# JeffWang987/MVSTER

Hardware: AMD Instinct MI355X
Metric: depth-maps/sec (DTU 512×640, 5-view, 4-stage) at 1/2/4/8 MI355X (higher is better)
Workload: dtype f32; 1 GPU; DTU mid 512x640, 5 views, 4-stage cascade 8/8/4/4 hyp, B=1 eval, 1 depth map(s) per step per GPU; launch=hipGraph replay, parallelism=replicas x1, depth_maps_in_flight_per_gpu=2

## Files before the change

include/mvster_hip.h:

```cpp
#ifndef MVSTER_HIP_H
#define MVSTER_HIP_H

#ifdef __cplusplus
extern "C" {
#endif

#define MVSTER_OK 0
#define MVSTER_ERR_NULL (-1)
#define MVSTER_ERR_SHAPE (-2)
#define MVSTER_ERR_UNSUPPORTED (-3)
#define MVSTER_ERR_LAUNCH (-4)

int mvster_relative_projection(const float* proj_matrices, float* rt, int B, int N, void* stream);

int mvster_relative_projection_multi(const float* const* proj_matrices, int nstage, float* rt, int B, int N,
                                     void* stream);

int mvster_pack_images(const float* const* imgs, int N, float* out, int B, int H, int W, void* stream);

int mvster_pack_images_u8(const unsigned char* imgs, float* out, int V, int H, int W, void* stream);

int mvster_load_pack_images_u8(const unsigned char* buf, long buf_bytes, const int* desc_host, const int* desc, const void* tables,
                               long table_words, float* out, unsigned char* out_u8, int V, int Hd, int Wd, void* stream);

// ... 59 lines not shown
                            float* partial, int B, int D, int h, int w, int CF, void* stream);

int mvster_upsample_bilinear(const float* in, float* out, int B, int hi, int wi, int ho, int wo, void* stream);

int mvster_upsample_bilinear_multi(const float* const* ins, float* const* outs, const int* his, const int* wis, int n, int B,
                                   int ho, int wo, void* stream);

int mvster_conv_mfma(const float* in, const float* wpk, const float* scale, const float* shift, const float* skip,
                     const float* zeros, const float* prob_w, const float* prob_b, float* out, const int* geom,
                     int ngeom, const long* woff, int cin, int mt, int nt, int variant, void* stream);

int mvster_conv_small(const float* in, const float* w, const float* scale, const float* shift, const float* skip,
                      float* out, int NB, int H, int W, int cin, int relu, void* stream);

int mvster_conv_narrow(const float* in, const float* w, const float* scale, const float* shift, const float* skip,
                       float* out, int NB, int H, int W, int cin, int relu, int mt, int wpc, void* stream);

int mvster_conv_narrow4(const float* in, const float* w, const float* scale, const float* shift, float* out, int NB, int H,
                        int W, int relu, int mt, int wpc, void* stream);

int mvster_conv_narrow_pair(const float* in, const float* w1, const float* scale1, const float* shift1, const float* w2,
                            const float* scale2, const float* shift2, float* out, int NB, int H, int W, int relu1, int relu2,
                            int wpc, void* stream);

int mvster_deconv_small(const float* in, const float* w, const float* scale, const float* shift, const float* skip,
                        const float* prob_w, const float* prob_b, float* out, int NB, int Hi, int Wi, int cin,
                        int cout, int relu, void* stream);

int mvster_deconv_select(const float* in, const float* w, const float* scale, const float* shift, const float* skip,
                         const float* prob_w, const float* prob_b, const float* hypo, float* attn, float* depth, float* conf,
                         float* inv_min, float* inv_max, float* logits_out, int B, int D, int Hi, int Wi, int cin, int relu,
                         float split_itv, void* stream);

int mvster_fpn_tail_gather(const float* G, const float* vb, float* P, float* workspace, int NB, int H, int W,
                           int CO, void* stream);

int mvster_fpn_tail_gather_bwd(const float* gP, float* gG, int NB, int H, int W, int CO, int pitch, void* stream);

int mvster_fpn_lateral_up(const float* x, const float* A, const float* bias, const float* q, float* out, int NB,
                          int H, int W, int CI, int CO, void* stream);

int mvster_fpn_tail_fused(const float* x, const float* A, const float* bias, const float* q, const float* vb, float* P,
                          int NB, int H, int W, int CI, void* stream);

int mvster_pack_conv_weights(const float* w, float* wpk, int cout, int cin, int cin_pad, int kd, int kh, int kw, long s_n,
                             long s_c, long s_z, long s_y, long s_x, int flip, void* stream);
// ... 128 lines not shown
```

mvster_amd/_lib.py:

```python
import ctypes
import os

_HERE = os.path.dirname(os.path.abspath(__file__))
LIB_PATH = os.environ.get("MVSTER_LIB") or os.path.join(_HERE, "csrc", "libmvster_hip.so")

ERR_NULL, ERR_SHAPE, ERR_UNSUPPORTED, ERR_LAUNCH = -1, -2, -3, -4
ERRORS = {-1: "NULL pointer", -2: "bad shape", -3: "unsupported channel/tile combination", -4: "kernel launch failed"}

_f = ctypes.c_void_p
_i = ctypes.c_int
_l = ctypes.c_long
_fl = ctypes.c_float

SIGNATURES = {
    "mvster_relative_projection": [_f, _f, _i, _i, _f],
    "mvster_relative_projection_multi": [_f, _i, _f, _i, _i, _f],
    "mvster_pack_images": [_f, _i, _f, _i, _i, _i, _f],
    "mvster_pack_images_u8": [_f, _f, _i, _i, _i, _f],
    "mvster_load_pack_images_u8": [_f, _l, _f, _f, _f, _l, _f, _f, _i, _i, _i, _f],
    "mvster_forward_prologue": [_f, _i, _f, _i, _i, _i, _f, _i, _f, _f, _i, _f, _i, _i, _i, _i, _f],
    "mvster_warp_agg_fwd": [_f, _f, _f, _f, _f, _f] + [_i] * 9 + [_l] * 3 + [_i, _i, _fl, _i, _f],
    "mvster_warp_agg_fwd_indexed": [_f, _f, _f, _f, _f, _f] + [_i] * 10 + [_fl, _i, _f],
    "mvster_warp_agg_fwd_counted": [_f, _f, _f, _f, _f, _f] + [_i] * 9 + [_l] * 3 + [_i, _i, _fl, _i, _f, _f],
    "mvster_warp_agg_fwd_indexed_counted": [_f, _f, _f, _f, _f, _f] + [_i] * 10 + [_fl, _i, _f, _f],
    "mvster_gather_views": [_f, _f, _f, _i, _i, _i, _l, _f],
    "mvster_warp_agg_fwd_sched": [_f] * 6 + [_i, _f, _f, _f] + [_i] * 9 + [_l] * 3 + [_i, _fl, _i, _f],
    "mvster_warp_agg_bwd": [_f] * 11 + [_i] * 9 + [_l] * 3 + [_i, _i, _fl, _f],
    "mvster_warp_agg_bwd_scratch": [_i] * 8 + [_f, _f],
    "mvster_warp_agg_bwd_sorted_scratch": [_i] * 8 + [_f, _f],
    "mvster_warp_agg_bwd_sorted": [_f] * 11 + [_i] * 9 + [_l] * 3 + [_i, _i, _fl, _f],
    "mvster_init_range": [_f, _i, _f, _i, _i, _i, _i, _i, _f],
    "mvster_schedule_inverse_range": [_f, _f, _f, _i, _i, _i, _i, _f],
    "mvster_schedule_range": [_f, _f, _f, _i, _i, _i, _i, _f],
    "mvster_select_depth": [_f, _f, _f, _f, _i, _f, _f, _f, _f, _f, _f, _f, _i, _i, _i, _i, _fl, _f],
    "mvster_select_depth_bwd": [_f, _f, _f, _f, _f, _f, _i, _i, _i, _i, _i, _f],
    "mvster_upsample_bilinear": [_f, _f, _i, _i, _i, _i, _i, _f],
    "mvster_upsample_bilinear_multi": [_f, _f, _f, _f, _i, _i, _i, _i, _f],
    "mvster_conv_mfma": [_f, _f, _f, _f, _f, _f, _f, _f, _f, _f, _i, _f, _i, _i, _i, _i, _f],
    "mvster_conv_small": [_f, _f, _f, _f, _f, _f, _i, _i, _i, _i, _i, _f],
    "mvster_conv_narrow": [_f, _f, _f, _f, _f, _f, _i, _i, _i, _i, _i, _i, _i, _f],
    "mvster_conv_narrow4": [_f, _f, _f, _f, _f, _i, _i, _i, _i, _i, _i, _f],
    "mvster_conv_narrow_pair": [_f, _f, _f, _f, _f, _f, _f, _f, _i, _i, _i, _i, _i, _i, _f],
    "mvster_deconv_select": [_f] * 14 + [_i] * 6 + [_fl, _f],
    "mvster_deconv_small": [_f, _f, _f, _f, _f, _f, _f, _f, _i, _i, _i, _i, _i, _i, _f],
    "mvster_fpn_tail_gather": [_f, _f, _f, _f, _i, _i, _i, _i, _f],
    "mvster_fpn_lateral_up": [_f, _f, _f, _f, _f, _i, _i, _i, _i, _i, _f],
    "mvster_fpn_tail_fused": [_f, _f, _f, _f, _f, _f, _i, _i, _i, _i, _f],
    "mvster_fpn_tail_gather_bwd": [_f, _f, _i, _i, _i, _i, _i, _f],
    "mvster_pack_conv_weights": [_f, _f] + [_i] * 6 + [_l] * 5 + [_i, _f],
    "mvster_pack_wino_weights": [_f, _f, _i, _i, _i, _i, _l, _l, _l, _l, _l, _i, _f],
    "mvster_pack_wino_batch": [_f, _i, _i, _f],
    "mvster_pack_conv_weights_classes": [_f, _f, _i, _i, _i, _i, _i, _f, _f, _f, _f],
    "mvster_conv_wgrad": [_f, _f, _f] + [_i] * 20 + [_f],
    "mvster_conv_wgrad_slots": [_i] * 12,
    "mvster_bn_relu_fwd": [_f, _f, _f, _f, _f, _l, _i, _i, _i, _f],
    "mvster_conv_wgrad_finish": [_f, _f] + [_i] * 10 + [_f],
    "mvster_bn_slots": [_l, _i, _i],
    "mvster_col_sum": [_f, _f, _f, _f, _l, _i, _f],
    "mvster_bn_train_slots": [_l, _i, _i],
    "mvster_bn_train_fwd": [_f] * 10 + [_l, _i, _i, _i, _fl, _fl, _f],
    "mvster_bn_train_bwd": [_f] * 7 + [_l, _i, _i, _i, _f],
    "mvster_conv_wgrad_finish_batch": [_f, _i, _f],
    "mvster_bn_relu_bwd_reduce": [_f] * 11 + [_l, _i, _i, _i, _f],
    "mvster_bn_relu_bwd_apply": [_f] * 8 + [_l, _i, _i, _i, _i, _f],
    "mvster_upsample2x_cl_fwd": [_f, _f, _i, _i, _i, _i, _f],
    "mvster_upsample2x_cl_bwd": [_f, _f, _i, _i, _i, _i, _f],
    "mvster_upsample2x_nearest_cl": [_f, _f, _i, _i, _i, _i, _i, _f],
    "mvster_sinkhorn": [_f, _f, _f, _f, _f, _i, _i, _l, _i, _fl, _f],
    "mvster_sinkhorn_continuous": [_f, _f, _f, _f, _f, _f, _i, _i, _l, _i, _fl, _f],
    "mvster_stage_loss_terms": [_f, _f, _f, _f, _f, _f, _i, _i, _l, _i, _f],
# ... 63 lines not shown
```

mvster_amd/conv_plan.py:

```python
import ctypes

import numpy as np
import torch

from . import _lib, ops

GEOM = ("B", "Di", "Hi", "Wi", "Do", "Ho", "Wo", "DoF", "HoF", "WoF", "sd", "sh", "sw", "cout", "ntile_total", "relu",
        "skip_mode", "osd", "osh", "osw", "nclass")
GEOM_CLASS = ("kd", "kh", "kw", "pd", "ph", "pw", "od", "oh", "ow", "nsteps")

SKIP_NONE, SKIP_ADD, SKIP_UPSAMPLE_ADD = 0, 1, 2


def _pack_gemm(wk):
    K, N = wk.shape
    Kp, Np = (K + 15) // 16 * 16, (N + 15) // 16 * 16
    full = wk.new_zeros(Kp, Np)
    full[:K, :N] = wk
    return full.view(Kp // 16, 4, 4, Np // 16, 16).permute(0, 3, 1, 4, 2).contiguous().view(-1), Kp // 16


def fold_bn(bn, cout, device):
    if bn is None:
        return torch.ones(cout, device=device), torch.zeros(cout, device=device)
# ... 48 lines not shown
    return _FAMILIES


def tuned_choice(layer, B, Di, Hi, Wi, skip_mode):
    import math
    sig = layer_signature(layer, B, Di, Hi, Wi, skip_mode)
    hit = _tuning().get(sig)
    if hit:
        return hit, "exact"
    if skip_mode == SKIP_ADD:
        hit = _tuning().get(sig[:-1] + "0")
        if hit:
            return hit, "exact (without skip)"
    lst = _families().get((sig[:sig.index("_", sig.index("_s") + 1)], skip_mode))
    if lst:
        lv, ld, lb = math.log2(max(1, B * Di * Hi * Wi)), math.log2(max(1, Di)), math.log2(max(1, B))
        d, val = min(((abs(e[0] - lv) + abs(e[1] - ld) + 0.25 * abs(e[2] - lb), e[3]) for e in lst), key=lambda t: t[0])
        if d <= FAMILY_REACH:
            return list(val), "family"
    return None, None


FUSE_TAIL = True
FUSE_SELECT = True
LDS_BUDGET = 12 * 256 * 16
FORCE_VARIANT = None
TPERS16_MIN_VOXELS = 40960
FUSE_CONV0 = True
NARROW_PAIR_WPC = 1
NARROW_PAIR_MIN_PIXELS = 512 * 14 * 64
NARROW_MIN_VOXELS = 64 * 256


def _lds_plan(B, Do, Ho, Wo, kernel, stride, ntile_total):
    kd, kh, kw = kernel
    if kw not in (3, 5) or Wo < 24:
        return None
    for mt in (4, 2):
        ty = 2 * mt
        patch = kd * ((ty - 1) * stride[1] + kh) * (31 * stride[2] + kw) * 64
        if patch > LDS_BUDGET or (mt == 4 and Ho < 6):
            continue
        blocks = -(-Wo // 32) * -(-Ho // ty) * Do * B
        nt = max(n for n in (4, 2, 1) if n <= ntile_total and ntile_total % n == 0)
        while nt > 1 and blocks * (ntile_total // nt) < 512:
            nt //= 2
# ... 578 lines not shown
        w3 = m.inner3.weight.detach().double()[:, :, 0, 0]
        b3 = m.inner3.bias.detach().double()
        self.tail_g, self.tail_c, self.tail_vb, wg4 = self._reassociate(m.out4, w3, b3)
        self.tail_a = (wg4 @ w2).float().contiguous()
        self.tail_ab = (wg4 @ b2).float().contiguous()

    @staticmethod
    def _reassociate(out, wi, bi):
        wo = out.weight.detach().double()
        co = wo.shape[0]
        wg = wo.permute(2, 3, 0, 1).reshape(9 * co, wo.shape[1])
        wc = torch.einsum("ocyx,ci->oiyx", wo, wi)
        g = ConvLayer(wg.float().reshape(9 * co, wo.shape[1], 1, 1), False, (1, 1), (0, 0))
        c = ConvLayer(wc.float(), False, (1, 1), (1, 1), bias=out.bias)
        vb = torch.einsum("ocyx,c->yxo", wo, bi).reshape(9, co).float().contiguous()
        return g, c, vb, wg

    @staticmethod
    def _seq(layers, x):
        for l in layers:
            x = l(x)
        return x

    def trunk(self, x):
        c0 = self._conv0(x)
        c1 = self._seq(self.conv1, c0)
        c2 = self._seq(self.conv2, c1)
        c3 = self._seq(self.conv3, c2)
        f1 = self.inner1(c2, skip=c3, skip_mode=SKIP_UPSAMPLE_ADD)
        return c0, c1, c3, f1

    def _conv0(self, x):
        a, b = self.conv0
        N, D, H, W, _ = x.shape
        if (FUSE_CONV0 and FORCE_VARIANT is None and a.w_small is not None and b.w_small is not None and a.cin == 4 and b.cin == 8
                and D == 1 and N * H * W >= NARROW_PAIR_MIN_PIXELS and x.is_cuda and a.w_small.device == x.device and x.is_contiguous() and x.dtype == torch.float32
                and hasattr(_lib.load(), "mvster_conv_narrow_pair")):
            out = torch.empty((N, 1, H, W, 8), device=x.device, dtype=torch.float32)
            rc = _lib.load().mvster_conv_narrow_pair(
                x.data_ptr(), a.w_small.data_ptr(), a.scale.data_ptr(), a.shift.data_ptr(), b.w_small.data_ptr(),
                b.scale.data_ptr(), b.shift.data_ptr(), out.data_ptr(), N, H, W, int(a.relu), int(b.relu), NARROW_PAIR_WPC, ops._stream())
            _lib.check(rc, "conv_narrow_pair")
            return out
        return self._seq(self.conv0, x)

    def coarse(self, c3, f1):
        return self.out1(c3), self.out2(f1)

    def head(self, x):
        c0, c1, c3, f1 = self.trunk(x)
        o1, o2 = self.coarse(c3, f1)
        return c0, c1, f1, o1, o2

    def tail(self, c0, c1, f1):
        return self.tail_mid(c0, c1, f1), self.tail_fine(c0, c1, f1)

    def tail_mid(self, c0, c1, f1):
        H, W = c0.shape[2], c0.shape[3]
        p3 = ops.fpn_tail_gather(self.mid_g(f1), self.mid_vb, H // 2, W // 2)
        return self.mid_c(c1, skip=p3, skip_mode=SKIP_ADD)

    def tail_fine(self, c0, c1, f1):
        H, W = c0.shape[2], c0.shape[3]
        q4 = self.tail_g(f1)
        p4 = ops.fpn_tail_fused(c1, self.tail_a, self.tail_ab, q4, self.tail_vb, H, W) if FUSE_TAIL else None
        if p4 is None:
            p4 = ops.fpn_tail_gather(ops.fpn_lateral_up(c1, self.tail_a, self.tail_ab, q4), self.tail_vb, H, W)
        return self.tail_c(c0, skip=p4, skip_mode=SKIP_ADD)

    def __call__(self, x):
        c0, c1, f1, o1, o2 = self.head(x)
        o3, o4 = self.tail(c0, c1, f1)
        return [o1, o2, o3, o4]
```

mvster_amd/csrc/conv_pers.hip:

```cpp
#include "conv_args.hpp"

namespace mvconv {
namespace {


#ifdef MVSTER_TIMELINE
__device__ unsigned long long* g_ptl = nullptr;
#define MV_PTL(k)                                                                                                       \
    do {                                                                                                                \
        __builtin_amdgcn_sched_barrier(0);                                                                              \
        if (g_ptl && lane == 0 && it < 16)                                                                              \
            g_ptl[(((size_t)(blockIdx.y * gridDim.x + blockIdx.x) * 4 + wave) * 16 + it) * 8 + (k)] =                    \
                (k) < 5 ? __builtin_amdgcn_s_memtime() : (k) == 5 ? __builtin_amdgcn_s_getreg(63492)                    \
                                                         : (k) == 6 ? __builtin_amdgcn_s_getreg(63508) : tile;          \
        __builtin_amdgcn_sched_barrier(0);                                                                              \
    } while (0)
#define MV_PPTL(k, v)                                                                                                   \
    do {                                                                                                                \
        __builtin_amdgcn_sched_barrier(0);                                                                              \
        if (g_ptl && lane == 0 && hp < 16)                                                                              \
            g_ptl[(((size_t)(blockIdx.y * gridDim.x + blockIdx.x) * 8 + wave8) * 16 + hp) * 4 + (k)] = (v);           \
        __builtin_amdgcn_sched_barrier(0);                                                                              \
    } while (0)
#else
// ... 977 lines not shown
                    const f32x4v k = __builtin_bit_cast(f32x4v, __builtin_amdgcn_raw_buffer_load_b128(skip_rsrc, off, 0, 0));
#pragma unroll
                    for (int j = 0; j < 4; ++j) v[j] += k[j];
                } else if (a.skip_mode == 2) {
                    const bool ok = n0 < (unsigned)a.cout && vox[mt] < mtot;
                    const unsigned c4 = n0 * 4u;
                    const f32x4v k00 = __builtin_bit_cast(f32x4v, __builtin_amdgcn_raw_buffer_load_b128(skip_rsrc, ok ? up[mt].o00 + c4 : 0x80000000u, 0, 0));
                    const f32x4v k01 = __builtin_bit_cast(f32x4v, __builtin_amdgcn_raw_buffer_load_b128(skip_rsrc, ok ? up[mt].o01 + c4 : 0x80000000u, 0, 0));
                    const f32x4v k10 = __builtin_bit_cast(f32x4v, __builtin_amdgcn_raw_buffer_load_b128(skip_rsrc, ok ? up[mt].o10 + c4 : 0x80000000u, 0, 0));
                    const f32x4v k11 = __builtin_bit_cast(f32x4v, __builtin_amdgcn_raw_buffer_load_b128(skip_rsrc, ok ? up[mt].o11 + c4 : 0x80000000u, 0, 0));
#pragma unroll
                    for (int j = 0; j < 4; ++j) v[j] = mv::bilerp(up[mt].ly, up[mt].lx, k00[j], k01[j], k10[j], k11[j]) + v[j];
                }
                __builtin_amdgcn_raw_buffer_store_b128(__builtin_bit_cast(u32x4v, v), out_rsrc, off, 0, MV_STORE_AUX);
            }
#pragma unroll
            for (int c = 0; c < NCH; ++c) Bv[c] = Bn[c];
        }
#pragma unroll
        for (int mt = 0; mt < MT; ++mt) {
            vox[mt] = voxn[mt];
#pragma unroll
            for (int c = 0; c < NCH; ++c) A[mt][c] = An[mt][c];
        }
    }
}


template <int MT, int NT, int KW, int SW, int NCH, int KD, bool WREG, int PF, bool SKIP, bool LD>
int launch_pers(const ConvArgs& a, int wpc, hipStream_t s) {
    using G = PersGeom<MT, KW, SW, KD>;
    constexpr int NTAP = KD * KW * KW;
    const size_t lds = (size_t)(2 * NCH * 2 * G::PLANE + 64 + (WREG ? 0 : NTAP * NCH * NT * 64)) * 16;
    if (lds > 160 * 1024) return MVSTER_ERR_UNSUPPORTED;
    auto kern = conv_pers_kernel<MT, NT, KW, SW, NCH, KD, WREG, PF, SKIP, LD>;
    static unsigned long attr_done = 0;
    if (lds > 64 * 1024 && !allow_big_lds(reinterpret_cast<const void*>(kern), attr_done)) return MVSTER_ERR_LAUNCH;
    const int g_num_cu = num_cus();
    if (g_num_cu <= 0) return MVSTER_ERR_LAUNCH;
    PersArgs p;
    if (!fill_pers_args(a, G::TY, p)) return MVSTER_ERR_UNSUPPORTED;
    const long ntiles = p.ntiles;
    p.prio = (wpc >> 4) & 1;
    wpc &= 15;
    int by_lds = (int)((160 * 1024) / lds);
    int per_cu = wpc > 0 ? wpc : (by_lds > 3 ? 3 : by_lds);
// ... 211 lines not shown
    if (mt == MT_ && nt == NT_ && kw == KW_ && sw == SW_ && nch == NCH_ && kd == KD_) {                            \
        if (ld) {                                                                                                  \
              \
            if constexpr (SW_ == 2)                                                                                \
                return a.skip_mode == 1 ? launch_pers<MT_, NT_, KW_, SW_, NCH_, KD_, WREG_, PF_, true, true>(a, wpc, s)   \
                                        : launch_pers<MT_, NT_, KW_, SW_, NCH_, KD_, WREG_, PF_, false, true>(a, wpc, s); \
            return MVSTER_ERR_UNSUPPORTED;                                                                         \
        }                                                                                                          \
        return a.skip_mode == 1 ? launch_pers<MT_, NT_, KW_, SW_, NCH_, KD_, WREG_, PF_, true, false>(a, wpc, s)   \
                                : launch_pers<MT_, NT_, KW_, SW_, NCH_, KD_, WREG_, PF_, false, false>(a, wpc, s);  \
    }
    MV_P(1, 3, 1, 1, 1, true, 2)
    MV_P(2, 3, 1, 2, 1, false, 1)
    MV_P(1, 3, 1, 2, 1, false, 1)
    MV_P(1, 3, 1, 4, 1, false, 1)
    MV_P(2, 5, 2, 1, 1, false, 1)
    MV_P(1, 3, 1, 1, 3, false, 2)
    MV_P(2, 3, 2, 1, 1, false, 1)
#undef MV_P
#undef MV_Q
    return MVSTER_ERR_UNSUPPORTED;
}

}
```

mvster_amd/graph.py:

```python
import collections

import torch


def _sample_layout(imgs, proj_matrices, depth_values):
    segs, off = [], 0
    for name, t in ([("img%d" % i, t) for i, t in enumerate(imgs)] + [("proj_" + k, proj_matrices[k]) for k in sorted(proj_matrices)]
                    + [("depth_values", depth_values)]):
        segs.append((name, off, tuple(t.shape)))
        off += (t.numel() + 63) // 64 * 64
    return segs, off


def pack_sample(imgs, proj_matrices, depth_values, pin=True):
    segs, total = _sample_layout(imgs, proj_matrices, depth_values)
    flat = torch.zeros(total, dtype=torch.float32)
    if pin:
        flat = flat.pin_memory()
    src = {("img%d" % i): t for i, t in enumerate(imgs)}
    src.update({"proj_" + k: v for k, v in proj_matrices.items()})
    src["depth_values"] = depth_values
    for name, off, shape in segs:
        flat[off:off + src[name].numel()].copy_(src[name].reshape(-1).float().cpu())
    return flat
# ... 116 lines not shown
        torch._foreach_copy_(new, self._src)
        out = {}
        for path, j in self._paths:
            if len(path) == 1:
                out[path[0]] = new[j]
            else:
                out.setdefault(path[0], {})[path[1]] = new[j]
        return {k: out[k] for k in self.outputs}


class ForwardCache:

    def __init__(self, capacity=4):
        self.capacity = capacity
        self.entries = collections.OrderedDict()
        self.stats = {"eager": 0, "captured": 0, "replayed": 0, "capture_failed": 0}
        self.disabled_keys = set()

    @staticmethod
    def key(model, imgs, proj_matrices, depth_values):
        im = imgs[0]
        from . import conv_plan, ops
        glob = (conv_plan.FORCE_VARIANT, conv_plan.FUSE_TAIL, conv_plan.FUSE_CONV0, conv_plan.NARROW_PAIR_WPC, conv_plan.FUSE_SELECT, conv_plan.LDS_BUDGET, conv_plan.NARROW_MIN_VOXELS,
                id(conv_plan._TUNING), ops.WGRAD_MAX_SLOTS)
        cfg = (glob, model.warp_variant, getattr(model, "fuse_hypotheses", None), getattr(model, "merge_launches", None), model.overlap_streams, float(model.attn_temp), model.attn_fuse_d, model.num_stage,
               tuple(model.stage_splits), tuple(model.depth_interals_ratio), tuple(model.group_cor_dim))
        return (im.device.index, len(imgs), tuple(im.shape), int(depth_values.shape[1]), tuple(sorted(proj_matrices.keys())), cfg)

    def clear(self):
        self.entries.clear()

    def __call__(self, model, imgs, proj_matrices, depth_values):
        key = self.key(model, imgs, proj_matrices, depth_values)
        if key in self.disabled_keys:
            self.stats["eager"] += 1
            return model._forward_eval(imgs, proj_matrices, depth_values)
        stamp = model._state_stamp()
        hit = self.entries.get(key)
        if hit is not None and hit[0] == stamp:
            self.entries.move_to_end(key)
            if hit[1] is None:
                try:
                    hit[1] = _CachedForward(model, imgs, proj_matrices, depth_values)
                    self.stats["captured"] += 1
                except RuntimeError as e:
                    import warnings
                    warnings.warn("mvster_amd: hipGraph capture of the eval forward failed for %r (%s): this shape stays on "
# ... 302 lines not shown
```

mvster_amd/net.py:

```python
import contextlib

import torch
import torch.nn as nn
import torch.nn.functional as F

from . import ops
from .conv_plan import FpnPlan, Reg2dPlan, Reg3dPlan
from .modules import FPN4, mono_depth_decoder, reg2d, reg3d


class _WarpAggPyr(torch.autograd.Function):

    @staticmethod
    def forward(ctx, pyr, B, rt, hypo, G, group_cor, attn_fuse_d, attn_temp):
        pyr = pyr.contiguous()
        ref_cl, src_cl = _WarpAggPyr._parts(pyr, B)
        out, wsum = ops.warp_agg_fwd_cl(ref_cl, src_cl, rt, hypo, G, group_cor, attn_fuse_d, attn_temp, want_wsum=True)
        ctx.save_for_backward(pyr, rt, hypo, out, wsum)
        ctx.cfg = (B, G, group_cor, attn_fuse_d, attn_temp)
        ctx.set_materialize_grads(False)
        return out, pyr[:B]

    @staticmethod
    def _parts(pyr, B):
        n, _, h, w, C = pyr.shape
        return pyr[:B].view(B, h, w, C), pyr[B:].view(n // B - 1, B, h, w, C)

    @staticmethod
    def backward(ctx, grad, grad_ref_maps):
# ... 196 lines not shown
                               "column)" % (tuple(depth_values.shape), B))
        if not imgs[0].is_cuda:
            raise RuntimeError("mvster_amd.MVS4net runs on MI355X only: move the model and inputs to the GPU "
                               "(there is no CPU fallback; the CPU oracle lives in oracle/ for tests)")

    @torch.no_grad()
    def _forward_eval(self, imgs, proj_matrices, depth_values, teacher=None, capture=None):
        N = len(imgs)
        B, _, H, W = imgs[0].shape
        dev = imgs[0].device
        fpn, regs = self._get_plans()
        depth_values = depth_values.to(dev, torch.float32)
        depth_interval = None
        if not self.inverse_depth:
            depth_interval = (depth_values[:, -1] - depth_values[:, 0]) / depth_values.size(1)
        names = ["stage%d" % (s + 1) for s in range(self.num_stage)]
        pms = [proj_matrices[n].to(dev, torch.float32) for n in names]
        hypo0 = None
        if self.merge_launches and (teacher is None or "stage1" not in teacher) and not self.fuse_hypotheses:
            packed, rts, hypo0 = ops.forward_prologue(imgs, pms, depth_values, self.stage_splits[0], H // 8, W // 8,
                                                      self.inverse_depth)
        else:
            packed, rts = ops.pack_images(imgs), ops.relative_projection_multi(pms)
        c0, c1, c3, f1 = fpn.trunk(packed)
        main = torch.cuda.current_stream()
        side = None
        if self.overlap_streams and self.num_stage > 2:
            side = self._side_streams.get(dev)
            if side is None:
                side = self._side_streams[dev] = torch.cuda.Stream(device=dev)
            side.wait_stream(main)
            with torch.cuda.stream(side):
                o3, o4 = fpn.tail(c0, c1, f1)
            o1, o2 = fpn.coarse(c3, f1)
        else:
            o1, o2 = fpn.coarse(c3, f1)
            o3, o4 = fpn.tail(c0, c1, f1) if self.num_stage > 2 else (None, None)
        join = None
        if side is not None:
            def join():
                main.wait_stream(side)
                if not torch.cuda.is_current_stream_capturing():
                    for t in (o3, o4):
                        t.record_stream(main)
        return self._cascade_eval([o1, o2, o3, o4], regs, N, B, H, W, rts, depth_values, depth_interval, hypo0=hypo0,
                                  teacher=teacher, capture=capture, join=join)

    @torch.no_grad()
    def _cascade_eval(self, pyramid, regs, N, B, H, W, rts, depth_values, depth_interval, hypo0=None, teacher=None,
                      capture=None, join=None, views=None, nsrc=None):
        outputs = {}
        prev = None
        for s in range(self.num_stage):
            name = "stage%d" % (s + 1)
            if s == 2 and join is not None:
                join()
            f = pyramid[s]
            if views is None:
                h, w, C = f.shape[2], f.shape[3], f.shape[4]
                f = f.view(N, B, h, w, C)
                ref_cl, src_cl = f[0], f[1:]
            else:
                h, w, C = f.shape[1], f.shape[2], f.shape[3]
                ref_cl = src_cl = None
            G = self.group_cor_dim[s] if self.group_cor else C
            rt = rts[s]
            cor = hypo = None
            if teacher is not None and name in teacher:
                hypo = teacher[name].contiguous()
            elif (views is None and nsrc is None and self.inverse_depth and self.group_cor and self.warp_variant == 0
                  and self.fuse_hypotheses):
                fused = ops.warp_agg_fwd_sched_cl(
                    ref_cl.contiguous(), src_cl.contiguous(), rt, G, self.stage_splits[s], self.attn_fuse_d, float(self.attn_temp),
                    inv_min=None if s == 0 else prev["inverse_min_depth"], inv_max=None if s == 0 else prev["inverse_max_depth"],
                    depth_values=depth_values.contiguous() if s == 0 else None)
                if fused is not None:
                    cor, hypo = fused
            if hypo is None and s == 0 and hypo0 is not None:
                hypo = hypo0
            if hypo is None:
# ... 163 lines not shown
```

mvster_amd/scan.py:

```python
import collections
import os
import weakref

import numpy as np
import torch

from . import formats, ops

ScanPlan = collections.namedtuple("ScanPlan", "ref_views view_table proj depth_values fusion_pairs source_counts")
ScanPlan.__doc__ = """Host planning of a scan (pure NumPy).  ``ref_views`` [R] view numbers that get a depth map, ``view_table``
int32 [R,nviews] (column 0 = the reference view, then its sources cut / padded as ``formats.eval_view_list`` does),
``proj`` dict stage1..4 -> [V,2,4,4] (``formats.stage_proj_matrices`` over ALL views: a sample's stack is
``proj[stage][view_table[r]]``), ``depth_values`` [R,ndv], ``fusion_pairs`` the pairs with sources, full source lists,
``source_counts`` int32 [R]: the sources row r runs with -- ``nviews - 1`` everywhere unless ``short_sources="fewer_views"``,
where a shorter list keeps its length and the unused slots of its row hold the reference view's own number (a valid
index with a finite projection stack, which the counted kernels never read)."""

SHORT_SOURCES = (None, "fewer_views")


def _check_short_sources(short_sources):
    if short_sources not in SHORT_SOURCES:
        raise RuntimeError("infer_scan: short_sources = %r (None or 'fewer_views')" % (short_sources,))

# ... 308 lines not shown
        at = {v: first + i for i, v in enumerate(views)}
        for r in rows:
            entries[r] = at[int(plan.view_table[r, 0])]
            entries[r, :1 + n] = [at[int(v)] for v in plan.view_table[r, :1 + n]]
        pages.append((1 + n, views, first))
        first += len(views)
    return entries, pages, first


def _run_fpn(model, runner, kind, dev_images, chunk, packed=None, V=None, pages=()):
    fpn = runner.plans[0]
    V = runner.V if V is None else V
    if packed is None and kind == "u8":
        packed = ops.pack_images_u8(dev_images)
    runs = 0
    for batch, views, first in [(chunk, list(range(V)), 0)] + list(pages):
        for a in range(0, len(views), batch):
            b = min(len(views), a + batch)
            idx = views[a:b] + [views[b - 1]] * (batch - (b - a))
            if kind == "u8":
                x = packed[idx[0]:idx[0] + batch] if idx == list(range(idx[0], idx[0] + batch)) else packed[idx]
            else:
                x = ops.pack_images([dev_images[i:i + 1] for i in idx])
            c0, c1, c3, f1 = fpn.trunk(x)
            levels = list(fpn.coarse(c3, f1)) + (list(fpn.tail(c0, c1, f1)) if model.num_stage > 2 else [None, None])
            for s in range(model.num_stage):
                runner.stores[s][first + a:first + b].copy_(levels[s][:b - a, 0])
            runs += 1
    return runs


@torch.no_grad()
def infer_scan(model, images, Ks, Es, depth_ranges, pairs, nviews=5, in_flight=2,
               keep=("depth", "photometric_confidence"), ndepths=192, fpn_chunk=None, max_store_bytes=None, view_ids=None,
               max_h=None, max_w=None, crop_rows=None, img_wh=None, depth_range_kind="min_interval", short_sources=None):
    _check_short_sources(short_sources)
    counted = short_sources == "fewer_views"
    inp = plan_inputs(images, Ks, max_h, max_w, crop_rows, img_wh, Es)
    kind, V, H, W, Ks = inp.kind, inp.V, inp.H, inp.W, inp.Ks
    if inp.exact_sources and not counted:
        _check_source_counts(_as_pairs(pairs, V), nviews, view_ids)
    plan = plan_scan(Ks, Es, depth_ranges, pairs, nviews, ndepths, depth_range_kind, short_sources)
    if in_flight < 1:
        raise RuntimeError("infer_scan: in_flight = %d" % in_flight)
    chunk = int(fpn_chunk or nviews)
    if not 1 <= chunk <= 16:
        raise RuntimeError("infer_scan: fpn_chunk = %d (1..16 images per FPN run)" % chunk)
    entries, pages, store_views = _short_entries(plan, V, nviews) if counted else (None, (), V)
# ... 244 lines not shown
```

Before: 1171 depth-maps/s.

## Fuse FPN top-down inner conv with tail 1x1 products in one kernel

Adds a persistent MFMA kernel that computes the inner1 1x1 conv with bilinear-upsampled skip add (f1), then reuses f1 from registers to compute the mid_g and tail_g 1x1 products (g3, q4). This replaces three separate conv launches and avoids re-reading f1 from global memory. It also moves the top-down computation onto the side stream, with main waiting on an event only when out2 needs f1, so the coarse out1 conv overlaps with the top-down work. The cost is a more complex schedule with lazy pyramid evaluation, and a kernel hard-coded to specific channel counts.

```diff
diff --git a/include/mvster_hip.h b/include/mvster_hip.h
--- a/include/mvster_hip.h
+++ b/include/mvster_hip.h
@@ -105,6 +105,11 @@
 int mvster_conv_narrow_pair(const float* in, const float* w1, const float* scale1, const float* shift1, const float* w2,
                             const float* scale2, const float* shift2, float* out, int NB, int H, int W, int relu1, int relu2,
                             int wpc, void* stream);
+
+int mvster_fpn_topdown_products(const float* c2, const float* c3, const float* w1, const float* scale1, const float* shift1,
+                                const float* w2, const float* scale2, const float* shift2, const float* w3,
+                                const float* scale3, const float* shift3, float* f1, float* g3, float* q4, int NB, int H,
+                                int W, int mt, int wpc, void* stream);
 
 int mvster_deconv_small(const float* in, const float* w, const float* scale, const float* shift, const float* skip,
                         const float* prob_w, const float* prob_b, float* out, int NB, int Hi, int Wi, int cin,
diff --git a/mvster_amd/_lib.py b/mvster_amd/_lib.py
--- a/mvster_amd/_lib.py
+++ b/mvster_amd/_lib.py
@@ -46,6 +46,7 @@
     "mvster_fpn_tail_gather": [_f, _f, _f, _f, _i, _i, _i, _i, _f],
     "mvster_fpn_lateral_up": [_f, _f, _f, _f, _f, _i, _i, _i, _i, _i, _f],
     "mvster_fpn_tail_fused": [_f, _f, _f, _f, _f, _f, _i, _i, _i, _i, _f],
+    "mvster_fpn_topdown_products": [_f] * 14 + [_i] * 5 + [_f],
     "mvster_fpn_tail_gather_bwd": [_f, _f, _i, _i, _i, _i, _i, _f],
     "mvster_pack_conv_weights": [_f, _f] + [_i] * 6 + [_l] * 5 + [_i, _f],
     "mvster_pack_wino_weights": [_f, _f, _i, _i, _i, _i, _l, _l, _l, _l, _l, _i, _f],
diff --git a/mvster_amd/conv_plan.py b/mvster_amd/conv_plan.py
--- a/mvster_amd/conv_plan.py
+++ b/mvster_amd/conv_plan.py
@@ -94,6 +94,10 @@
 
 
 FUSE_TAIL = True
+FUSE_TOPDOWN = True
+TOPDOWN_MT = 1
+TOPDOWN_WPC = 18
+TOPDOWN_ON_SIDE = True
 FUSE_SELECT = True
 LDS_BUDGET = 12 * 256 * 16
 FORCE_VARIANT = None
@@ -718,13 +722,57 @@
             x = l(x)
         return x
 
-    def trunk(self, x):
+    def trunk(self, x, tail=False):
+        c0, c1, c2, c3 = self.bottom_up(x)
+        return (c0, c1, c3) + self.topdown(c2, c3, tail)
+
+    def bottom_up(self, x):
         c0 = self._conv0(x)
         c1 = self._seq(self.conv1, c0)
         c2 = self._seq(self.conv2, c1)
         c3 = self._seq(self.conv3, c2)
-        f1 = self.inner1(c2, skip=c3, skip_mode=SKIP_UPSAMPLE_ADD)
-        return c0, c1, c3, f1
+        return c0, c1, c2, c3
+
+    def topdown(self, c2, c3, tail=False):
+        fused = self._topdown(c2, c3) if tail else None
+        if fused is not None:
+            return fused
+        return self.inner1(c2, skip=c3, skip_mode=SKIP_UPSAMPLE_ADD), None
+
+    def topdown_fuses(self, c2, c3):
+        a, g, t = self.inner1, self.mid_g, self.tail_g
+        if not FUSE_TOPDOWN or FORCE_VARIANT is not None:
+            return False
+        for x in (c2, c3):
+            if not x.is_cuda or x.dtype != torch.float32 or not x.is_contiguous() or x.device != a.wpk.device:
+                return False
+        if not hasattr(_lib.load(), "mvster_fpn_topdown_products"):
+            return False
+        N, D, H, W, C = c2.shape
+        if (D != 1 or (C, a.cin, a.cout, g.cin, g.cout, t.cin, t.cout) != (32, 32, 64, 64, 144, 64, 72) or a.relu or g.relu or t.relu
+                or tuple(c3.shape) != (N, 1, H // 2, W // 2, 64)):
+            return False
+        if H % 2 or W % 2 or N * H * W * 144 * 4 >= 1 << 31:
+            return False
+        return all((layer._geom(N, 1, H, W, sm)[4] & 0xff) in (0, 6)
+                   for layer, sm in ((a, SKIP_UPSAMPLE_ADD), (g, SKIP_NONE), (t, SKIP_NONE)))
+
+    def _topdown(self, c2, c3):
+        if not self.topdown_fuses(c2, c3):
+            return None
+        a, g, t = self.inner1, self.mid_g, self.tail_g
+        N, _, H, W, _ = c2.shape
+        f1 = torch.empty((N, 1, H, W, 64), device=c2.device, dtype=torch.float32)
+        g3 = torch.empty((N, 1, H, W, 144), device=c2.device, dtype=torch.float32)
+        q4 = torch.empty((N, 1, H, W, 72), device=c2.device, dtype=torch.float32)
+        rc = _lib.load().mvster_fpn_topdown_products(
+            c2.data_ptr(), c3.data_ptr(), a.wpk.data_ptr(), a.scale.data_ptr(), a.shift.data_ptr(), g.wpk.data_ptr(),
+            g.scale.data_ptr(), g.shift.data_ptr(), t.wpk.data_ptr(), t.scale.data_ptr(), t.shift.data_ptr(), f1.data_ptr(),
+            g3.data_ptr(), q4.data_ptr(), N, H, W, TOPDOWN_MT, TOPDOWN_WPC, ops._stream())
+        if rc == _lib.ERR_UNSUPPORTED:
+            return None
+        _lib.check(rc, "fpn_topdown_products")
+        return f1, (g3, q4)
 
     def _conv0(self, x):
         a, b = self.conv0
@@ -743,28 +791,30 @@
     def coarse(self, c3, f1):
         return self.out1(c3), self.out2(f1)
 
-    def head(self, x):
-        c0, c1, c3, f1 = self.trunk(x)
+    def head(self, x, tail=False):
+        c0, c1, c3, f1, taps = self.trunk(x, tail=tail)
         o1, o2 = self.coarse(c3, f1)
-        return c0, c1, f1, o1, o2
-
-    def tail(self, c0, c1, f1):
-        return self.tail_mid(c0, c1, f1), self.tail_fine(c0, c1, f1)
-
-    def tail_mid(self, c0, c1, f1):
+        return c0, c1, f1, o1, o2, taps
+
+    def tail(self, c0, c1, f1, taps=None):
+        g3, q4 = taps if taps is not None else (None, None)
+        return self.tail_mid(c0, c1, f1, g3), self.tail_fine(c0, c1, f1, q4)
+
+    def tail_mid(self, c0, c1, f1, g3=None):
         H, W = c0.shape[2], c0.shape[3]
-        p3 = ops.fpn_tail_gather(self.mid_g(f1), self.mid_vb, H // 2, W // 2)
+        p3 = ops.fpn_tail_gather(self.mid_g(f1) if g3 is None else g3, self.mid_vb, H // 2, W // 2)
         return self.mid_c(c1, skip=p3, skip_mode=SKIP_ADD)
 
-    def tail_fine(self, c0, c1, f1):
+    def tail_fine(self, c0, c1, f1, q4=None):
         H, W = c0.shape[2], c0.shape[3]
-        q4 = self.tail_g(f1)
+        if q4 is None:
+            q4 = self.tail_g(f1)
         p4 = ops.fpn_tail_fused(c1, self.tail_a, self.tail_ab, q4, self.tail_vb, H, W) if FUSE_TAIL else None
         if p4 is None:
             p4 = ops.fpn_tail_gather(ops.fpn_lateral_up(c1, self.tail_a, self.tail_ab, q4), self.tail_vb, H, W)
         return self.tail_c(c0, skip=p4, skip_mode=SKIP_ADD)
 
     def __call__(self, x):
-        c0, c1, f1, o1, o2 = self.head(x)
-        o3, o4 = self.tail(c0, c1, f1)
+        c0, c1, f1, o1, o2, taps = self.head(x, tail=True)
+        o3, o4 = self.tail(c0, c1, f1, taps)
         return [o1, o2, o3, o4]
diff --git a/mvster_amd/csrc/conv_pers.hip b/mvster_amd/csrc/conv_pers.hip
--- a/mvster_amd/csrc/conv_pers.hip
+++ b/mvster_amd/csrc/conv_pers.hip
@@ -1023,6 +1023,178 @@
             vox[mt] = voxn[mt];
 #pragma unroll
             for (int c = 0; c < NCH; ++c) A[mt][c] = An[mt][c];
+        }
+    }
+}
+
+struct TopdownArgs {
+    const float *c2, *c3;
+    const float *w[3], *scale[3], *shift[3];
+    float *f1, *g3, *q4;
+    int H, W;
+    unsigned ngroups, mtot;
+    unsigned div_mul[2], div_shr[2];
+};
+
+constexpr int kTdC1 = 64, kTdC2 = 144, kTdC3 = 72;
+constexpr int kTdNt1 = 4, kTdNt2 = 9, kTdNt3 = 5;
+constexpr int kTdW1 = 0, kTdW2 = kTdW1 + 2 * kTdNt1 * 64, kTdW3 = kTdW2 + 4 * kTdNt2 * 64;
+constexpr int kTdSs = kTdW3 + 4 * kTdNt3 * 64;
+constexpr int kTdLds = (kTdSs + 2 * 4 * (kTdNt1 + kTdNt2 + kTdNt3)) * 16;
+
+template <int MT>
+__global__ void __launch_bounds__(256, 2) fpn_topdown_kernel(TopdownArgs t) {
+    extern __shared__ __attribute__((aligned(16))) float lds_raw[];
+    f32x4v* const wl = reinterpret_cast<f32x4v*>(lds_raw);
+    f32x4v* const ssl = wl + kTdSs;
+    const int lane = threadIdx.x & 63;
+    const int wave = __builtin_amdgcn_readfirstlane(threadIdx.x >> 6);
+    const int lm = lane & 15, lq = lane >> 4;
+    const unsigned mtot = t.mtot;
+    const __amdgpu_buffer_rsrc_t in_rsrc =
+        __builtin_amdgcn_make_buffer_rsrc(const_cast<float*>(t.c2), (short)0, (int)(mtot * 32u * 4u), 0x00020000);
+    const __amdgpu_buffer_rsrc_t skip_rsrc =
+        __builtin_amdgcn_make_buffer_rsrc(const_cast<float*>(t.c3), (short)0, (int)(mtot * kTdC1), 0x00020000);
+    const __amdgpu_buffer_rsrc_t f1_rsrc = __builtin_amdgcn_make_buffer_rsrc(t.f1, (short)0, (int)(mtot * kTdC1 * 4u), 0x00020000);
+    const __amdgpu_buffer_rsrc_t g3_rsrc = __builtin_amdgcn_make_buffer_rsrc(t.g3, (short)0, (int)(mtot * kTdC2 * 4u), 0x00020000);
+    const __amdgpu_buffer_rsrc_t q4_rsrc = __builtin_amdgcn_make_buffer_rsrc(t.q4, (short)0, (int)(mtot * kTdC3 * 4u), 0x00020000);
+    {
+        const int wbase[3] = {kTdW1, kTdW2, kTdW3}, nblk[3] = {2 * kTdNt1, 4 * kTdNt2, 4 * kTdNt3}, ntl[3] = {kTdNt1, kTdNt2, kTdNt3};
+        int ss = 0;
+#pragma unroll
+        for (int l = 0; l < 3; ++l) {
+            const __amdgpu_buffer_rsrc_t w_rsrc =
+                __builtin_amdgcn_make_buffer_rsrc(const_cast<float*>(t.w[l]), (short)0, nblk[l] * 1024, 0x00020000);
+            for (int i = wave; i < nblk[l]; i += 4) {
+                const unsigned off = (unsigned)(i * 1024 + lane * 16);
+                f32x4v* const dst = wl + wbase[l] + i * 64;
+                __builtin_amdgcn_raw_ptr_buffer_load_lds(w_rsrc, (lds_void*)dst, 16, off, 0, 0, 0);
+            }
+            for (int i = threadIdx.x; i < ntl[l] * 4; i += 256) {
+                ssl[ss + i] = *reinterpret_cast<const f32x4v*>(t.scale[l] + i * 4);
+                ssl[ss + ntl[l] * 4 + i] = *reinterpret_cast<const f32x4v*>(t.shift[l] + i * 4);
+            }
+            ss += 2 * 4 * ntl[l];
+        }
+    }
+    constexpr int kSs1 = 0, kSs2 = 2 * 4 * kTdNt1, kSs3 = kSs2 + 2 * 4 * kTdNt2;
+    auto load_group = [&](unsigned g, f32x4v (&A)[MT][2], unsigned (&vox)[MT]) {
+#pragma unroll
+        for (int mt = 0; mt < MT; ++mt) {
+            const unsigned m = ((g * 4 + wave) * MT + mt) * 16 + lm;
+            vox[mt] = m;
+#pragma unroll
+            for (int c = 0; c < 2; ++c) {
+                const unsigned off = m < mtot ? (m * 32 + c * 16 + lq * 4) * 4u : 0x80000000u;
+                A[mt][c] = __builtin_bit_cast(f32x4v, __builtin_amdgcn_raw_buffer_load_b128(in_rsrc, off, 0, 0));
+            }
+        }
+    };
+    f32x4v A[MT][2], An[MT][2];
+    unsigned vox[MT], voxn[MT];
+    unsigned g = blockIdx.x;
+    if (g < t.ngroups) load_group(g, A, vox);
+    __syncthreads();
+    for (; g < t.ngroups; g += gridDim.x) {
+        const unsigned gn = g + gridDim.x < t.ngroups ? g + gridDim.x : g;
+        load_group(gn, An, voxn);
+        struct Up {
+            unsigned o00, o01, o10, o11;
+            mv::Lerp ly, lx;
+        } up[MT];
+        {
+            const int hh = t.H / 2, wh = t.W / 2;
+#pragma unroll
+            for (int mt = 0; mt < MT; ++mt) {
+                const unsigned m = vox[mt] < mtot ? vox[mt] : 0u;
+                const unsigned q = fast_div(m, (unsigned)t.W, t.div_mul[0], t.div_shr[0]);
+                const int ox = (int)(m - q * (unsigned)t.W);
+                const unsigned b = fast_div(q, (unsigned)t.H, t.div_mul[1], t.div_shr[1]);
+                const int oy = (int)(q - b * (unsigned)t.H);
+                up[mt].ly = mv::make_lerp(oy, hh, t.H);
+                up[mt].lx = mv::make_lerp(ox, wh, t.W);
+                const unsigned base = b * (unsigned)(hh * wh);
+                up[mt].o00 = (base + up[mt].ly.i0 * wh + up[mt].lx.i0) * (kTdC1 * 4u);
+                up[mt].o01 = (base + up[mt].ly.i0 * wh + up[mt].lx.i1) * (kTdC1 * 4u);
+                up[mt].o10 = (base + up[mt].ly.i1 * wh + up[mt].lx.i0) * (kTdC1 * 4u);
+                up[mt].o11 = (base + up[mt].ly.i1 * wh + up[mt].lx.i1) * (kTdC1 * 4u);
+            }
+        }
+        f32x4v F[MT][kTdNt1];
+#pragma unroll
+        for (int nt = 0; nt < kTdNt1; ++nt) {
+            const f32x4v B0 = wl[kTdW1 + nt * 64 + lane], B1 = wl[kTdW1 + (kTdNt1 + nt) * 64 + lane];
+            const f32x4v sc = ssl[kSs1 + nt * 4 + lq], sh = ssl[kSs1 + kTdNt1 * 4 + nt * 4 + lq];
+            f32x4v acc[MT];
+#pragma unroll
+            for (int mt = 0; mt < MT; ++mt) acc[mt] = (f32x4v){0.f, 0.f, 0.f, 0.f};
+#pragma unroll
+            for (int j = 0; j < 4; ++j)
+#pragma unroll
+                for (int mt = 0; mt < MT; ++mt) acc[mt] = __builtin_amdgcn_mfma_f32_16x16x4f32(B0[j], A[mt][0][j], acc[mt], 0, 0, 0);
+#pragma unroll
+            for (int j = 0; j < 4; ++j)
+#pragma unroll
+                for (int mt = 0; mt < MT; ++mt) acc[mt] = __builtin_amdgcn_mfma_f32_16x16x4f32(B1[j], A[mt][1][j], acc[mt], 0, 0, 0);
+            const unsigned c4 = (unsigned)(nt * 16 + lq * 4) * 4u;
+#pragma unroll
+            for (int mt = 0; mt < MT; ++mt) {
+                const bool ok = vox[mt] < mtot;
+                f32x4v v = acc[mt];
+#pragma unroll
+                for (int j = 0; j < 4; ++j) v[j] = fmaf(v[j], sc[j], sh[j]);
+                const f32x4v k00 = __builtin_bit_cast(f32x4v, __builtin_amdgcn_raw_buffer_load_b128(skip_rsrc, ok ? up[mt].o00 + c4 : 0x80000000u, 0, 0));
+                const f32x4v k01 = __builtin_bit_cast(f32x4v, __builtin_amdgcn_raw_buffer_load_b128(skip_rsrc, ok ? up[mt].o01 + c4 : 0x80000000u, 0, 0));
+                const f32x4v k10 = __builtin_bit_cast(f32x4v, __builtin_amdgcn_raw_buffer_load_b128(skip_rsrc, ok ? up[mt].o10 + c4 : 0x80000000u, 0, 0));
+                const f32x4v k11 = __builtin_bit_cast(f32x4v, __builtin_amdgcn_raw_buffer_load_b128(skip_rsrc, ok ? up[mt].o11 + c4 : 0x80000000u, 0, 0));
+#pragma unroll
+                for (int j = 0; j < 4; ++j) v[j] = mv::bilerp(up[mt].ly, up[mt].lx, k00[j], k01[j], k10[j], k11[j]) + v[j];
+                __builtin_amdgcn_raw_buffer_store_b128(__builtin_bit_cast(u32x4v, v), f1_rsrc, ok ? vox[mt] * (kTdC1 * 4u) + c4 : 0x80000000u, 0,
+                                                       MV_STORE_AUX);
+                F[mt][nt] = v;
+            }
+        }
+        auto tap_product = [&](const f32x4v* w, const f32x4v* ss, int ntile, unsigned cout, const __amdgpu_buffer_rsrc_t& rsrc) {
+            f32x4v Bv[4];
+#pragma unroll
+            for (int c = 0; c < 4; ++c) Bv[c] = w[(c * ntile) * 64 + lane];
+#pragma nounroll
+            for (int nt = 0; nt < ntile; ++nt) {
+                f32x4v Bn[4];
+                const int ntn = nt + 1 < ntile ? nt + 1 : nt;
+#pragma unroll
+                for (int c = 0; c < 4; ++c) Bn[c] = w[(c * ntile + ntn) * 64 + lane];
+                const f32x4v sc = ss[nt * 4 + lq], sh = ss[ntile * 4 + nt * 4 + lq];
+                f32x4v acc[MT];
+#pragma unroll
+                for (int mt = 0; mt < MT; ++mt) acc[mt] = (f32x4v){0.f, 0.f, 0.f, 0.f};
+#pragma unroll
+                for (int c = 0; c < 4; ++c)
+#pragma unroll
+                    for (int j = 0; j < 4; ++j)
+#pragma unroll
+                        for (int mt = 0; mt < MT; ++mt)
+                            acc[mt] = __builtin_amdgcn_mfma_f32_16x16x4f32(Bv[c][j], F[mt][c][j], acc[mt], 0, 0, 0);
+                const unsigned n0 = (unsigned)(nt * 16 + lq * 4);
+#pragma unroll
+                for (int mt = 0; mt < MT; ++mt) {
+                    const unsigned off = (n0 < cout && vox[mt] < mtot) ? vox[mt] * (cout * 4u) + n0 * 4u : 0x80000000u;
+                    f32x4v v = acc[mt];
+#pragma unroll
+                    for (int j = 0; j < 4; ++j) v[j] = fmaf(v[j], sc[j], sh[j]);
+                    __builtin_amdgcn_raw_buffer_store_b128(__builtin_bit_cast(u32x4v, v), rsrc, off, 0, MV_STORE_AUX);
+                }
+#pragma unroll
+                for (int c = 0; c < 4; ++c) Bv[c] = Bn[c];
+            }
+        };
+        tap_product(wl + kTdW2, ssl + kSs2, kTdNt2, kTdC2, g3_rsrc);
+        tap_product(wl + kTdW3, ssl + kSs3, kTdNt3, kTdC3, q4_rsrc);
+#pragma unroll
+        for (int mt = 0; mt < MT; ++mt) {
+            vox[mt] = voxn[mt];
+#pragma unroll
+            for (int c = 0; c < 2; ++c) A[mt][c] = An[mt][c];
         }
     }
 }
@@ -1280,4 +1452,52 @@
     return MVSTER_ERR_UNSUPPORTED;
 }
 
-}
+namespace {
+template <int MT>
+int launch_topdown(TopdownArgs t, int wpc, hipStream_t s) {
+    auto kern = fpn_topdown_kernel<MT>;
+    static unsigned long attr_done = 0;
+    if (!allow_big_lds(reinterpret_cast<const void*>(kern), attr_done)) return MVSTER_ERR_LAUNCH;
+    const int ncu = num_cus();
+    if (ncu <= 0) return MVSTER_ERR_LAUNCH;
+    const long ngroups = ((long)t.mtot + 64 * MT - 1) / (64 * MT);
+    int per_cu = (wpc & 15) > 0 ? (wpc & 15) : 2;
+    if (per_cu > 2) per_cu = 2;
+    const long gmax = (long)ncu * per_cu;
+    const long rounds = (ngroups + gmax - 1) / gmax;
+    const long gx = (wpc & 16) ? (ngroups < gmax ? ngroups : gmax) : (ngroups + rounds - 1) / rounds;
+    t.ngroups = (unsigned)ngroups;
+    MV_NOTE_KERNEL("fpn_topdown_kernel<%d>", MT);
+    hipLaunchKernelGGL(kern, dim3((unsigned)gx), dim3(256), kTdLds, s, t);
+    return mv_check_launch();
+}
+}
+
+}
+
+extern "C" int mvster_fpn_topdown_products(const float* c2, const float* c3, const float* w1, const float* scale1, const float* shift1,
+                                           const float* w2, const float* scale2, const float* shift2, const float* w3,
+                                           const float* scale3, const float* shift3, float* f1, float* g3, float* q4, int NB,
+                                           int H, int W, int mt, int wpc, void* stream) {
+    using namespace mvconv;
+    if (!c2 || !c3 || !w1 || !scale1 || !shift1 || !w2 || !scale2 || !shift2 || !w3 || !scale3 || !shift3 || !f1 || !g3 || !q4)
+        return MVSTER_ERR_NULL;
+    if (NB <= 0 || H <= 0 || W <= 0) return MVSTER_ERR_SHAPE;
+    if ((H & 1) || (W & 1)) return MVSTER_ERR_UNSUPPORTED;
+    const long mtot = (long)NB * H * W;
+    if (mtot * kTdC2 * 4 >= (1L << 31)) return MVSTER_ERR_UNSUPPORTED;
+    TopdownArgs t;
+    t.c2 = c2; t.c3 = c3;
+    t.w[0] = w1; t.scale[0] = scale1; t.shift[0] = shift1;
+    t.w[1] = w2; t.scale[1] = scale2; t.shift[1] = shift2;
+    t.w[2] = w3; t.scale[2] = scale3; t.shift[2] = shift3;
+    t.f1 = f1; t.g3 = g3; t.q4 = q4;
+    t.H = H; t.W = W;
+    t.mtot = (unsigned)mtot;
+    t.ngroups = 0;
+    find_divisor((unsigned)W, t.div_mul[0], t.div_shr[0]);
+    find_divisor((unsigned)H, t.div_mul[1], t.div_shr[1]);
+    if (mt == 1) return launch_topdown<1>(t, wpc, (hipStream_t)stream);
+    if (mt == 2) return launch_topdown<2>(t, wpc, (hipStream_t)stream);
+    return MVSTER_ERR_UNSUPPORTED;
+}
diff --git a/mvster_amd/graph.py b/mvster_amd/graph.py
--- a/mvster_amd/graph.py
+++ b/mvster_amd/graph.py
@@ -162,7 +162,7 @@
         im = imgs[0]
         from . import conv_plan, ops
         glob = (conv_plan.FORCE_VARIANT, conv_plan.FUSE_TAIL, conv_plan.FUSE_CONV0, conv_plan.NARROW_PAIR_WPC, conv_plan.FUSE_SELECT, conv_plan.LDS_BUDGET, conv_plan.NARROW_MIN_VOXELS,
-                id(conv_plan._TUNING), ops.WGRAD_MAX_SLOTS)
+                id(conv_plan._TUNING), ops.WGRAD_MAX_SLOTS, conv_plan.FUSE_TOPDOWN, conv_plan.TOPDOWN_MT, conv_plan.TOPDOWN_WPC, conv_plan.TOPDOWN_ON_SIDE)
         cfg = (glob, model.warp_variant, getattr(model, "fuse_hypotheses", None), getattr(model, "merge_launches", None), model.overlap_streams, float(model.attn_temp), model.attn_fuse_d, model.num_stage,
                tuple(model.stage_splits), tuple(model.depth_interals_ratio), tuple(model.group_cor_dim))
         return (im.device.index, len(imgs), tuple(im.shape), int(depth_values.shape[1]), tuple(sorted(proj_matrices.keys())), cfg)
diff --git a/mvster_amd/net.py b/mvster_amd/net.py
--- a/mvster_amd/net.py
+++ b/mvster_amd/net.py
@@ -4,7 +4,7 @@
 import torch.nn as nn
 import torch.nn.functional as F
 
-from . import ops
+from . import conv_plan, ops
 from .conv_plan import FpnPlan, Reg2dPlan, Reg3dPlan
 from .modules import FPN4, mono_depth_decoder, reg2d, reg3d
 
@@ -247,20 +247,37 @@
                                                       self.inverse_depth)
         else:
             packed, rts = ops.pack_images(imgs), ops.relative_projection_multi(pms)
-        c0, c1, c3, f1 = fpn.trunk(packed)
         main = torch.cuda.current_stream()
         side = None
         if self.overlap_streams and self.num_stage > 2:
             side = self._side_streams.get(dev)
             if side is None:
                 side = self._side_streams[dev] = torch.cuda.Stream(device=dev)
+        c0, c1, c2, c3 = fpn.bottom_up(packed)
+        if side is not None and conv_plan.TOPDOWN_ON_SIDE and fpn.topdown_fuses(c2, c3):
             side.wait_stream(main)
             with torch.cuda.stream(side):
-                o3, o4 = fpn.tail(c0, c1, f1)
+                f1, taps = fpn.topdown(c2, c3, tail=True)
+                have_f1 = torch.cuda.Event()
+                have_f1.record(side)
+                o3, o4 = fpn.tail(c0, c1, f1, taps)
+            o1 = fpn.out1(c3)
+
+            def o2():
+                main.wait_event(have_f1)
+                if not torch.cuda.is_current_stream_capturing():
+                    f1.record_stream(main)
+                return fpn.out2(f1)
+        elif side is not None:
+            f1, taps = fpn.topdown(c2, c3, tail=True)
+            side.wait_stream(main)
+            with torch.cuda.stream(side):
+                o3, o4 = fpn.tail(c0, c1, f1, taps)
             o1, o2 = fpn.coarse(c3, f1)
         else:
+            f1, taps = fpn.topdown(c2, c3, tail=self.num_stage > 2)
             o1, o2 = fpn.coarse(c3, f1)
-            o3, o4 = fpn.tail(c0, c1, f1) if self.num_stage > 2 else (None, None)
+            o3, o4 = fpn.tail(c0, c1, f1, taps) if self.num_stage > 2 else (None, None)
         join = None
         if side is not None:
             def join():
@@ -281,6 +298,8 @@
             if s == 2 and join is not None:
                 join()
             f = pyramid[s]
+            if callable(f):
+                f = pyramid[s] = f()
             if views is None:
                 h, w, C = f.shape[2], f.shape[3], f.shape[4]
                 f = f.view(N, B, h, w, C)
diff --git a/mvster_amd/scan.py b/mvster_amd/scan.py
--- a/mvster_amd/scan.py
+++ b/mvster_amd/scan.py
@@ -354,8 +354,8 @@
                 x = packed[idx[0]:idx[0] + batch] if idx == list(range(idx[0], idx[0] + batch)) else packed[idx]
             else:
                 x = ops.pack_images([dev_images[i:i + 1] for i in idx])
-            c0, c1, c3, f1 = fpn.trunk(x)
-            levels = list(fpn.coarse(c3, f1)) + (list(fpn.tail(c0, c1, f1)) if model.num_stage > 2 else [None, None])
+            c0, c1, c3, f1, taps = fpn.trunk(x, tail=model.num_stage > 2)
+            levels = list(fpn.coarse(c3, f1)) + (list(fpn.tail(c0, c1, f1, taps)) if model.num_stage > 2 else [None, None])
             for s in range(model.num_stage):
                 runner.stores[s][first + a:first + b].copy_(levels[s][:b - a, 0])
             runs += 1
```

Result: no change. 1179 depth-maps/s (median of 3 runs) (+0.7%).
